# jabhinav/RetinaNet-for-Table-Detection

Hardware: AMD Instinct MI355X
Metric: images/sec RetinaNet R50-FPN 800x1333 inference (higher is better)
Workload: dtype bf16; 1 GPU; ResNet50-FPN RetinaNet inference 800x1333 bf16 batch 8/GPU incl. decode+NMS (BASELINE.json configs[1]); batch_per_gpu=8, anchors_per_image=200700, parallelism=dp1 (images sharded, no collective), batches_in_flight=2

## Files before the change

retinanet-for-table-detection_amd/csrc/rtn_conv_halon.hip:

```cpp
#include "rtn_internal.h"
#include "rtn_device.h"

namespace {

typedef __attribute__((ext_vector_type(8))) __bf16 bf16x8;
typedef __attribute__((ext_vector_type(4))) float f32x4;
typedef __attribute__((ext_vector_type(4))) unsigned u32x4;

constexpr unsigned HN_OOB = 0xFFFFFF00u;
constexpr int HN_THREADS = 512;
constexpr int HN_R = 256, HN_TM = HN_R - 3;
constexpr unsigned HN_HALO = 32768, HN_ZERO_ROW = (HN_R - 1) * 128u;

template <int NF>
struct HNCfg {
    static constexpr int BR = 48 * NF;
    static constexpr int BP = BR / 8;
    static constexpr int BPW = (BP + 7) / 8;
    static constexpr unsigned STAGE = HN_HALO + BR * 128u;
    static constexpr unsigned DUMP = 3 * STAGE;
    static constexpr int LDS = 3 * (int)STAGE + 1024;
    static constexpr int PP = 4 + BPW;
};

struct HNGroup {
    const char* in;
    char* out;
    unsigned in_bytes, out_bytes;
    int Hin, Win, M, tile_begin;
    int in_row_stride_b;
    int cells;
    unsigned out_img_stride, out_off;
    float inv_cells, inv_w;
};

struct HNParams {
    HNGroup g[RTN_MAX_GROUPS];
    const char* w;
    const float* bias;
    unsigned w_bytes;
    int ngroups, ntiles;
    int N, Kbytes, nchunk, pad_t, pad_l, relu, sigmoid, out_ld, pix_b, vec, xcd, kh_fast;
};

__device__ __forceinline__ void dma16(const i32x4& srd, unsigned voff, unsigned soff, unsigned lds_addr) {
    unsigned keep;
    const unsigned la = (unsigned)__builtin_amdgcn_readfirstlane((int)lds_addr), so = (unsigned)__builtin_amdgcn_readfirstlane((int)soff);
    asm volatile("s_mov_b32 %0, m0\n\ts_mov_b32 m0, %2\n\ts_nop 0\n\tbuffer_load_dwordx4 %1, %3, %4 offen lds\n\ts_mov_b32 m0, %0"
                 : "=&s"(keep)
                 : "v"(voff), "s"(la), "s"(srd), "s"(so)
                 : "memory");
}

#define RTN_STORE_GUARD(V) asm volatile("s_nop 3" :: "v"(V.x), "v"(V.y), "v"(V.z), "v"(V.w));
#define RTN_STORE_GUARD1(V) asm volatile("s_nop 1" :: "v"(V));

template <int NF>
__global__ __launch_bounds__(HN_THREADS, 2) void conv_halon_kernel(const HNParams p) {
    typedef HNCfg<NF> Cfg;
    extern __shared__ __attribute__((aligned(16))) char lds[];

    const int t = threadIdx.x, lane = t & 63;
    const int wave = __builtin_amdgcn_readfirstlane(t >> 6);
    const int lr = lane >> 3, sc = (lane & 7) ^ lr;
    const int lrow = lane & 15, kq = lane >> 4;
    const unsigned lds_base = (unsigned)(size_t)(__attribute__((address_space(3))) char*)lds;
    const int nchunk = p.nchunk;
    const int G = 3 * nchunk;
    const i32x4 w_srd = make_srd(p.w, p.w_bytes);

    unsigned wvoff[Cfg::BPW];
#pragma unroll
    for (int d = 0; d < Cfg::BPW; ++d) {
        const int row = (d * 8 + wave) * 8 + lr;
        const int kw = row / (16 * NF), n = row - kw * (16 * NF);
        wvoff[d] = row < Cfg::BR ? (unsigned)n * (unsigned)p.Kbytes + (unsigned)(kw * nchunk * 128) + (unsigned)sc * 16u : HN_OOB;
    }

    unsigned hbase[4];
    int hiy[4];
    i32x4 in_srd = w_srd;
    int st_Hin = 1, st_row_b = 0;
    auto stage_tile = [&](int T) {
        if (T >= p.ntiles) {
#pragma unroll
            for (int i = 0; i < 4; ++i) { hiy[i] = -(1 << 28); hbase[i] = 0; }
            return;
        }
        int gi = 0;
#pragma unroll
        for (int i = 1; i < RTN_MAX_GROUPS; ++i)
            if (i < p.ngroups && T >= p.g[i].tile_begin) gi = i;
        const HNGroup& Gs = p.g[gi];
        const int m0 = (T - Gs.tile_begin) * HN_TM;
        in_srd = make_srd(Gs.in, Gs.in_bytes);
        st_Hin = Gs.Hin;
        st_row_b = Gs.in_row_stride_b;
#pragma unroll
        for (int i = 0; i < 4; ++i) {
            const int h = (i * 8 + wave) * 8 + lr;
            const int f = m0 + h - p.pad_l;
            if (h < HN_R - 1 && f >= 0 && f < Gs.M) {
                int b, rem, y, x;
                divmod24(f, Gs.cells, Gs.inv_cells, b, rem);
                divmod24(rem, Gs.Win, Gs.inv_w, y, x);
                hiy[i] = y;
                hbase[i] = (unsigned)f * (unsigned)p.pix_b + (unsigned)sc * 16u;
            } else {
                hiy[i] = -(1 << 28);
                hbase[i] = 0;
            }
        }
    };
    auto tile_of = [&](int v) {
        if (v >= p.ntiles || !p.xcd) return v;
        const int x = v & 7, j = v >> 3, base = p.ntiles >> 3, rem = p.ntiles & 7;
        return x * base + (x < rem ? x : rem) + j;
    };
    int st_v = blockIdx.x, st_kh = 0, st_cc = 0;
    unsigned st_ring = 0;
#define HN_ISSUE(I)                                                                                            \
    if ((I) < 4) {                                                                                             \
        const int dy_ = st_kh - p.pad_t;                                                                       \
        const unsigned delta_ = (unsigned)(dy_ * st_row_b + st_cc * 128);                                      \
        const bool ok_ = (unsigned)(hiy[(I) & 3] + dy_) < (unsigned)st_Hin;                                    \
        dma16(in_srd, ok_ ? hbase[(I) & 3] + delta_ : HN_OOB, 0u, lds_base + st_ring + (unsigned)(wave * 1024 + ((I) & 3) * 8192)); \
    } else if ((I) < Cfg::PP) {                                                                                \
        constexpr int d_ = (I) >= 4 && (I) - 4 < Cfg::BPW ? (I) - 4 : 0;                                       \
        const unsigned kcol_ = (unsigned)((st_kh * 3 * nchunk + st_cc) * 128);                                 \
        const int P_ = d_ * 8 + wave;                                                                          \
        dma16(w_srd, wvoff[d_], kcol_, lds_base + (P_ < Cfg::BP ? st_ring + HN_HALO + (unsigned)P_ * 1024u : Cfg::DUMP)); \
    }
    auto advance_stage = [&]() {
        st_ring = st_ring == 2 * Cfg::STAGE ? 0u : st_ring + Cfg::STAGE;
        if (p.kh_fast) {
            if (++st_kh == 3) {
                st_kh = 0;
                if (++st_cc == nchunk) { st_cc = 0; st_v += (int)gridDim.x; stage_tile(tile_of(st_v)); }
            }
        } else if (++st_cc == nchunk) {
            st_cc = 0;
            if (++st_kh == 3) {
                st_kh = 0;
                st_v += (int)gridDim.x;
                stage_tile(tile_of(st_v));
            }
        }
    };
    auto issue_stage = [&]() {
        HN_ISSUE(0) HN_ISSUE(1) HN_ISSUE(2) HN_ISSUE(3) HN_ISSUE(4) HN_ISSUE(5) HN_ISSUE(6)
        advance_stage();
    };

    f32x4 bias4[NF];
#pragma unroll
    for (int f = 0; f < NF; ++f) {
        bias4[f] = (f32x4){0.f, 0.f, 0.f, 0.f};
        if (p.bias) bias4[f] = *reinterpret_cast<const f32x4*>(p.bias + 16 * f + 4 * kq);
    }
    const unsigned w_lane = HN_HALO + (unsigned)(lrow * 128 + ((kq ^ (lrow & 7)) << 4));

    stage_tile(tile_of(st_v));
    issue_stage();
    issue_stage();

    unsigned c_ring = 0;
    int cv = blockIdx.x;
    bool first = true;
    while (cv < p.ntiles) {
        const int tile = tile_of(cv);
        int gi = 0;
#pragma unroll
        for (int i = 1; i < RTN_MAX_GROUPS; ++i)
            if (i < p.ngroups && tile >= p.g[i].tile_begin) gi = i;
        const HNGroup& Gc = p.g[gi];
        const int m0 = (tile - Gc.tile_begin) * HN_TM;
        unsigned arow[3][2];
        unsigned obase[2];
#pragma unroll
        for (int i = 0; i < 2; ++i) {
            const int rloc = wave * 32 + i * 16 + lrow;
            const int m = m0 + rloc;
            const int mc = m < Gc.M ? m : Gc.M - 1;
            int b, rem, y, x;
            divmod24(mc, Gc.cells, Gc.inv_cells, b, rem);
            divmod24(rem, Gc.Win, Gc.inv_w, y, x);
#pragma unroll
            for (int kw = 0; kw < 3; ++kw) {
                const int rr = rloc + kw;
                const bool off = rloc >= HN_TM || (unsigned)(x + kw - p.pad_l) >= (unsigned)Gc.Win;
                arow[kw][i] = off ? HN_ZERO_ROW : (unsigned)(rr * 128 + ((kq ^ (rr & 7)) << 4));
            }
            obase[i] = (rloc < HN_TM && m < Gc.M) ? (unsigned)b * Gc.out_img_stride + Gc.out_off + (unsigned)rem * (unsigned)p.out_ld : HN_OOB;
        }
        f32x4 acc[2][NF];
#pragma unroll
        for (int i = 0; i < 2; ++i)
#pragma unroll
            for (int f = 0; f < NF; ++f) acc[i][f] = bias4[f];

#pragma unroll 1
        for (int g = 0; g < G; ++g) {
            if (g == 0 && !first) {
                if (p.vec) asm volatile("s_waitcnt vmcnt(%0)" :: "n"(Cfg::PP + 2 * NF) : "memory");
                else       asm volatile("s_waitcnt vmcnt(%0)" :: "n"(Cfg::PP + 8 * NF) : "memory");
            } else {
                asm volatile("s_waitcnt vmcnt(%0)" :: "n"(Cfg::PP) : "memory");
            }
            __builtin_amdgcn_s_barrier();
            const char* sb = lds + c_ring;
            uint4 fx[2][2], fw[2][NF];
#define HN_READ(STEP, SET)                                                                                     \
            {                                                                                                  \
                const int kw_ = ((STEP) >> 1) % 3;                                                             \
                const unsigned ks_ = ((STEP) & 1) * 64u;                                                       \
                _Pragma("unroll") for (int i = 0; i < 2; ++i) fx[SET][i] = *reinterpret_cast<const uint4*>(sb + (arow[kw_][i] ^ ks_)); \
                _Pragma("unroll") for (int f = 0; f < NF; ++f)                                                 \
                    fw[SET][f] = *reinterpret_cast<const uint4*>(sb + ((w_lane ^ ks_) + (unsigned)((kw_ * NF + f) * 2048))); \
            }
#define HN_STEP(STEP)                                                                                          \
            {                                                                                                  \
                if ((STEP) + 1 < 6) HN_READ((STEP) + 1, ((STEP) + 1) & 1)                                      \
                if (0 * 6 / Cfg::PP == (STEP)) { HN_ISSUE(0) }                                                 \
                if (1 * 6 / Cfg::PP == (STEP)) { HN_ISSUE(1) }                                                 \
                if (2 * 6 / Cfg::PP == (STEP)) { HN_ISSUE(2) }                                                 \
                if (3 * 6 / Cfg::PP == (STEP)) { HN_ISSUE(3) }                                                 \
                if (4 * 6 / Cfg::PP == (STEP)) { HN_ISSUE(4) }                                                 \
                if (5 < Cfg::PP && 5 * 6 / Cfg::PP == (STEP)) { HN_ISSUE(5) }                                  \
                if (6 < Cfg::PP && 6 * 6 / Cfg::PP == (STEP)) { HN_ISSUE(6) }                                  \
                _Pragma("unroll") for (int f = 0; f < NF; ++f)                                                 \
                    _Pragma("unroll") for (int i = 0; i < 2; ++i)                                              \
                        acc[i][f] = __builtin_amdgcn_mfma_f32_16x16x32_bf16(__builtin_bit_cast(bf16x8, fw[(STEP) & 1][f]),      \
                                                                           __builtin_bit_cast(bf16x8, fx[(STEP) & 1][i]), acc[i][f], 0, 0, 0); \
            }
            HN_READ(0, 0)
            HN_STEP(0) HN_STEP(1) HN_STEP(2) HN_STEP(3) HN_STEP(4) HN_STEP(5)
#undef HN_STEP
#undef HN_READ
            advance_stage();
            c_ring = c_ring == 2 * Cfg::STAGE ? 0u : c_ring + Cfg::STAGE;
        }
        {
            const __amdgpu_buffer_rsrc_t out_rsrc = __builtin_amdgcn_make_buffer_rsrc(
                (void*)Gc.out, 0, (int)__builtin_amdgcn_readfirstlane((int)Gc.out_bytes), 0x00020000);
#pragma unroll
            for (int i = 0; i < 2; ++i)
#pragma unroll
                for (int f = 0; f < NF; ++f) {
                    f32x4 v = acc[i][f];
                    if (p.relu) {
#pragma unroll
                        for (int r = 0; r < 4; ++r) v[r] = v[r] > 0.f ? v[r] : 0.f;
                    }
                    if (p.sigmoid) {
#pragma unroll
                        for (int r = 0; r < 4; ++r) v[r] = 1.0f / (1.0f + expf(-v[r]));
                    }
                    const int ch0 = 16 * f + 4 * kq;
                    const int cnt = p.N - ch0;
                    if (p.vec) {
                        const unsigned off = (obase[i] != HN_OOB && cnt >= 4) ? (obase[i] + (unsigned)ch0) * 4u : HN_OOB;
                        u32x4 o = __builtin_bit_cast(u32x4, v);
                        __builtin_amdgcn_raw_buffer_store_b128(o, out_rsrc, (int)off, 0, 0);
                        RTN_STORE_GUARD(o)
                    } else {
#pragma unroll
                        for (int r = 0; r < 4; ++r) {
                            const unsigned off = (obase[i] != HN_OOB && r < cnt) ? (obase[i] + (unsigned)(ch0 + r)) * 4u : HN_OOB;
                            const unsigned o = __float_as_uint(v[r]);
                            __builtin_amdgcn_raw_buffer_store_b32(o, out_rsrc, (int)off, 0, 0);
                            RTN_STORE_GUARD1(o)
                        }
                    }
                }
        }
        cv += (int)gridDim.x;
        first = false;
    }
    asm volatile("s_waitcnt vmcnt(0)" ::: "memory");
#undef HN_ISSUE
}

}

int rtn_conv_halon_try(rtn_handle_t h, const rtn_conv_desc_t* d, int grid_limit, bool forced) {
    if (d->dtype != RTN_BF16) return 1;
    if (d->KW != 3 || d->KH != 3 || d->sy != 1 || d->sx != 1) return 1;
    if (!(d->flags & RTN_CONV_OUT_F32) || (d->flags & ~(RTN_CONV_OUT_F32 | RTN_CONV_RELU | RTN_CONV_SIGMOID))) return 1;
    if (d->N < 1 || d->N > 48 || d->out_ld < d->N) return 1;
    const int nf = (d->N + 15) / 16;
    if (d->w_rows < 16 * nf) return 1;
    if (d->Crun != d->pix_stride || (d->Crun * 2) % 128 || d->Crun <= 0) return 1;
    if (d->pad_l < 0 || d->pad_l >= 3 || d->pad_t < 0 || d->pad_t >= 3) return 1;
    if (((uintptr_t)d->w & 15) || ((uintptr_t)d->bias & 15)) return 1;
    const int nchunk = d->Crun * 2 / 128;
    const long long Kbytes = 9ll * d->Crun * 2;
    if (Kbytes * d->w_rows >= 0xFFFFFF00ll) return 1;
    HNParams p;
    memset(&p, 0, sizeof(p));
    const int cus = h->num_cus > 0 ? h->num_cus : 256;
    long long tiles = 0;
    bool vec = d->N % 4 == 0 && d->out_ld % 4 == 0;
    for (int i = 0; i < d->ngroups; ++i) {
        const rtn_conv_group_t& s = d->g[i];
        if (s.Hin != s.Hout || s.Win != s.Wout || s.in_row_stride != (long long)s.Win * d->pix_stride ||
            s.in_img_stride != (long long)s.Hin * s.in_row_stride) return 1;
        const long long cells = (long long)s.Hout * s.Wout, M = cells * d->batch;
        if (s.out_step > 1 || s.out_off < 0 || M >= (1ll << 24) || M < 1) return 1;
        if (!s.in || !s.out || ((uintptr_t)s.in & 15) || ((uintptr_t)s.out & 3)) return 1;
        if (s.in_elems < M * d->Crun || s.in_elems * 2 >= 0xFFFFFF00ll || s.out_elems * 4 >= 0xFFFFFF00ll) return 1;
        if (s.out_img_stride < 0 || (d->batch - 1) * s.out_img_stride + s.out_off + (cells - 1) * d->out_ld + d->N > s.out_elems) return 1;
        if (((uintptr_t)s.out & 15) || s.out_img_stride % 4 || s.out_off % 4) vec = false;
        HNGroup& g = p.g[i];
        g.in = (const char*)s.in;
        g.out = (char*)s.out;
        g.in_bytes = (unsigned)(s.in_elems * 2);
        g.out_bytes = (unsigned)(s.out_elems * 4);
        g.Hin = s.Hin; g.Win = s.Win; g.M = (int)M;
        g.cells = (int)cells;
        g.tile_begin = (int)tiles;
        g.in_row_stride_b = (int)(s.in_row_stride * 2);
        g.out_img_stride = (unsigned)s.out_img_stride;
        g.out_off = (unsigned)s.out_off;
        g.inv_cells = 1.0f / (float)cells;
        g.inv_w = 1.0f / (float)s.Win;
        tiles += (M + HN_TM - 1) / HN_TM;
    }
    if (tiles < 1 || tiles > 0x3fffffff) return 1;
    if (!forced && tiles * 4 < cus) return 1;
    p.w = (const char*)d->w;
    p.bias = d->bias;
    p.w_bytes = (unsigned)(Kbytes * d->w_rows);
    p.ngroups = d->ngroups;
    p.ntiles = (int)tiles;
    p.N = d->N;
    p.Kbytes = (int)Kbytes;
    p.nchunk = nchunk;
    p.pad_t = d->pad_t; p.pad_l = d->pad_l;
    p.relu = (d->flags & RTN_CONV_RELU) ? 1 : 0;
    p.sigmoid = (d->flags & RTN_CONV_SIGMOID) ? 1 : 0;
    p.out_ld = d->out_ld;
    p.pix_b = d->pix_stride * 2;
    p.vec = vec ? 1 : 0;
    p.xcd = 1;
    p.kh_fast = 1;
    int grid = cus;
    if (grid_limit > 0 && grid_limit < grid) grid = grid_limit;
    if (grid > p.ntiles) grid = p.ntiles;
    const dim3 gdim((unsigned)grid), bdim(HN_THREADS);
    const int lrc = nf == 1 ? rtn_launch_lds<conv_halon_kernel<1>>(h, gdim, bdim, HNCfg<1>::LDS, HNCfg<1>::LDS, p)
                  : nf == 2 ? rtn_launch_lds<conv_halon_kernel<2>>(h, gdim, bdim, HNCfg<2>::LDS, HNCfg<2>::LDS, p)
                            : rtn_launch_lds<conv_halon_kernel<3>>(h, gdim, bdim, HNCfg<3>::LDS, HNCfg<3>::LDS, p);
    if (lrc != RTN_OK) return lrc;
    RTN_CHECK_LAUNCH(h, "conv_halon_kernel");
    return RTN_OK;
}
```

Measured before the change: 2441 images/sec.

## Add 2D-tiled halo conv kernel for 3x3 head convolutions

Adds a new 3x3 convolution kernel that tiles the output as 2D blocks (8x32 or 6x42 pixels) with a small halo, in place of 1D row strips that stage a large halo. Per output tile the kernel double-buffers the halo input across channel chunks and streams the weights per kh-row into LDS, overlapping DMA with the MFMA work. The aim is to cut redundant halo loads and LDS footprint, which could allow two blocks per CU. It is enabled by default through an env flag, and it adds complex index math plus the risk of partially filled tiles at the image edges.

Result: no change. 2440 images/sec (-0.0%).

```diff
diff --git a/retinanet-for-table-detection_amd/csrc/rtn_conv_halon.hip b/retinanet-for-table-detection_amd/csrc/rtn_conv_halon.hip
--- a/retinanet-for-table-detection_amd/csrc/rtn_conv_halon.hip
+++ b/retinanet-for-table-detection_amd/csrc/rtn_conv_halon.hip
@@ -32,6 +32,8 @@
     int cells;
     unsigned out_img_stride, out_off;
     float inv_cells, inv_w;
+    int th, tw, txn, tpi;
+    float inv_tw, inv_hw, inv_txn, inv_tpi;
 };
 
 struct HNParams {
@@ -281,6 +283,255 @@
 #undef HN_ISSUE
 }
 
+constexpr int H2_HJ = 6;
+constexpr int H2_PIECES = 44;
+constexpr unsigned H2_HALO = H2_PIECES * 1024u;
+struct H2Shape { int th, tw; };
+constexpr H2Shape H2_SHAPES[] = {{8, 32}, {6, 42}};
+constexpr bool h2_shapes_fit() {
+    for (const H2Shape& s : H2_SHAPES)
+        if (s.th * s.tw > 256 || (s.th + 2) * (s.tw + 2) > H2_PIECES * 8) return false;
+    return true;
+}
+static_assert(h2_shapes_fit(), "a tile is at most 256 pixels and its halo at most one halo slot");
+
+template <int NF>
+struct H2Cfg {
+    static constexpr int BR = 48 * NF, BP = BR / 8, BPW = (BP + 7) / 8;
+    static constexpr unsigned WST = BR * 128u;
+    static constexpr unsigned WBASE = 2 * H2_HALO;
+    static constexpr unsigned DUMP = WBASE + 3 * WST;
+    static constexpr int LDS = (int)DUMP + 1024;
+};
+
+template <int NF>
+__global__ __launch_bounds__(HN_THREADS, 2) void conv_halon2d_kernel(const HNParams p) {
+    typedef H2Cfg<NF> Cfg;
+    extern __shared__ __attribute__((aligned(16))) char lds[];
+
+    const int t = threadIdx.x, lane = t & 63;
+    const int wave = __builtin_amdgcn_readfirstlane(t >> 6);
+    const int lr = lane >> 3, sc = (lane & 7) ^ lr;
+    const int lrow = lane & 15, kq = lane >> 4;
+    const unsigned lds_base = (unsigned)(size_t)(__attribute__((address_space(3))) char*)lds;
+    const int nchunk = p.nchunk;
+    const i32x4 w_srd = make_srd(p.w, p.w_bytes);
+
+    unsigned wvoff[Cfg::BPW];
+#pragma unroll
+    for (int d = 0; d < Cfg::BPW; ++d) {
+        const int row = (d * 8 + wave) * 8 + lr;
+        const int kw = row / (16 * NF), n = row - kw * (16 * NF);
+        wvoff[d] = row < Cfg::BR ? (unsigned)n * (unsigned)p.Kbytes + (unsigned)(kw * nchunk * 128) + (unsigned)sc * 16u : HN_OOB;
+    }
+
+    unsigned hbase[H2_HJ];
+    i32x4 in_srd = w_srd;
+    auto stage_tile = [&](int T) {
+        if (T >= p.ntiles) {
+#pragma unroll
+            for (int j = 0; j < H2_HJ; ++j) hbase[j] = HN_OOB;
+            return;
+        }
+        int gi = 0;
+#pragma unroll
+        for (int i = 1; i < RTN_MAX_GROUPS; ++i)
+            if (i < p.ngroups && T >= p.g[i].tile_begin) gi = i;
+        const HNGroup& Gs = p.g[gi];
+        int b, r, ty, tx;
+        divmod24(T - Gs.tile_begin, Gs.tpi, Gs.inv_tpi, b, r);
+        divmod24(r, Gs.txn, Gs.inv_txn, ty, tx);
+        const int y0 = ty * Gs.th - p.pad_t, x0 = tx * Gs.tw - p.pad_l, hw = Gs.tw + 2, hrows = (Gs.th + 2) * hw;
+        in_srd = make_srd(Gs.in, Gs.in_bytes);
+#pragma unroll
+        for (int j = 0; j < H2_HJ; ++j) {
+            const int h = (j * 8 + wave) * 8 + lr;
+            int hy, hx;
+            divmod24(h, hw, Gs.inv_hw, hy, hx);
+            const int iy = y0 + hy, ix = x0 + hx;
+            const bool ok = h < hrows && (unsigned)iy < (unsigned)Gs.Hin && (unsigned)ix < (unsigned)Gs.Win;
+            hbase[j] = ok ? (unsigned)((b * Gs.Hin + iy) * Gs.Win + ix) * (unsigned)p.pix_b + (unsigned)sc * 16u : HN_OOB;
+        }
+    };
+    auto tile_of = [&](int v) {
+        if (v >= p.ntiles || !p.xcd) return v;
+        const int x = v & 7, j = v >> 3, base = p.ntiles >> 3, rem = p.ntiles & 7;
+        return x * base + (x < rem ? x : rem) + j;
+    };
+#define H2_HALO_PIECE(J, CC, HB)                                                                               \
+    {                                                                                                          \
+        const int P_ = (J) * 8 + wave;                                                                         \
+        dma16(in_srd, hbase[J] != HN_OOB ? hbase[J] + (unsigned)((CC) * 128) : HN_OOB, 0u,                     \
+              lds_base + (P_ < H2_PIECES ? (HB) + (unsigned)P_ * 1024u : Cfg::DUMP));                          \
+    }
+#define H2_W_PIECE(D, FKH, FCC)                                                                                \
+    {                                                                                                          \
+        const unsigned kcol_ = (unsigned)(((FKH) * 3 * nchunk + (FCC)) * 128);                                 \
+        const int P_ = (D) * 8 + wave;                                                                         \
+        dma16(w_srd, wvoff[D], kcol_, lds_base + (P_ < Cfg::BP ? Cfg::WBASE + (FKH) * Cfg::WST + (unsigned)P_ * 1024u : Cfg::DUMP)); \
+    }
+#define H2_ISSUE(KH, I)                                                                                        \
+    if ((KH) < 2 && (I) < 3) {                                                                                 \
+        constexpr int j_ = ((KH) < 2 && (I) < 3) ? (KH) * 3 + (I) : 0;                                         \
+        H2_HALO_PIECE(j_, ncc, hb ^ H2_HALO)                                                                   \
+    } else if ((I) - ((KH) < 2 ? 3 : 0) < Cfg::BPW) {                                                          \
+        constexpr int d0_ = (I) - ((KH) < 2 ? 3 : 0);                                                          \
+        constexpr int d_ = d0_ >= 0 && d0_ < Cfg::BPW ? d0_ : 0;                                               \
+        constexpr int fkh_ = ((KH) + 2) % 3;                                                                   \
+        const int fcc_ = (KH) == 0 ? c : ncc;                                                                  \
+        H2_W_PIECE(d_, fkh_, fcc_)                                                                             \
+    }
+
+    f32x4 bias4[NF];
+#pragma unroll
+    for (int f = 0; f < NF; ++f) {
+        bias4[f] = (f32x4){0.f, 0.f, 0.f, 0.f};
+        if (p.bias) bias4[f] = *reinterpret_cast<const f32x4*>(p.bias + 16 * f + 4 * kq);
+    }
+    const unsigned w_lane = Cfg::WBASE + (unsigned)(lrow * 128 + ((kq ^ (lrow & 7)) << 4));
+
+    int st_v = blockIdx.x;
+    unsigned hb = 0;
+    stage_tile(tile_of(st_v));
+    H2_HALO_PIECE(0, 0, 0u) H2_HALO_PIECE(1, 0, 0u) H2_HALO_PIECE(2, 0, 0u)
+    H2_HALO_PIECE(3, 0, 0u) H2_HALO_PIECE(4, 0, 0u) H2_HALO_PIECE(5, 0, 0u)
+#pragma unroll
+    for (int d = 0; d < Cfg::BPW; ++d) H2_W_PIECE(d, 0, 0)
+#pragma unroll
+    for (int d = 0; d < Cfg::BPW; ++d) H2_W_PIECE(d, 1, 0)
+
+    int cv = blockIdx.x;
+    bool first = true;
+    while (cv < p.ntiles) {
+        const int tile = tile_of(cv);
+        int gi = 0;
+#pragma unroll
+        for (int i = 1; i < RTN_MAX_GROUPS; ++i)
+            if (i < p.ngroups && tile >= p.g[i].tile_begin) gi = i;
+        const HNGroup& Gc = p.g[gi];
+        int tb, trem, ty, tx;
+        divmod24(tile - Gc.tile_begin, Gc.tpi, Gc.inv_tpi, tb, trem);
+        divmod24(trem, Gc.txn, Gc.inv_txn, ty, tx);
+        const int hw = Gc.tw + 2, tpix = Gc.th * Gc.tw;
+        unsigned arow[3][3][2];
+        unsigned obase[2];
+#pragma unroll
+        for (int i = 0; i < 2; ++i) {
+            const int rloc = wave * 32 + i * 16 + lrow;
+            const int rc = rloc < tpix ? rloc : tpix - 1;
+            int y, x;
+            divmod24(rc, Gc.tw, Gc.inv_tw, y, x);
+            const int oy = ty * Gc.th + y, ox = tx * Gc.tw + x;
+#pragma unroll
+            for (int kh = 0; kh < 3; ++kh)
+#pragma unroll
+                for (int kw = 0; kw < 3; ++kw) {
+                    const int hp = (y + kh) * hw + x + kw;
+                    arow[kh][kw][i] = (unsigned)(hp * 128 + ((kq ^ (hp & 7)) << 4));
+                }
+            obase[i] = (rloc < tpix && oy < Gc.Hin && ox < Gc.Win)
+                           ? (unsigned)tb * Gc.out_img_stride + Gc.out_off + (unsigned)(oy * Gc.Win + ox) * (unsigned)p.out_ld : HN_OOB;
+        }
+        f32x4 acc[2][NF];
+#pragma unroll
+        for (int i = 0; i < 2; ++i)
+#pragma unroll
+            for (int f = 0; f < NF; ++f) acc[i][f] = bias4[f];
+
+#pragma unroll 1
+        for (int c = 0; c < nchunk; ++c) {
+            int ncc = c + 1;
+            if (ncc == nchunk) { ncc = 0; st_v += (int)gridDim.x; stage_tile(tile_of(st_v)); }
+            const char* hbuf = lds + hb;
+#define H2_READ(KH, STEP, SET)                                                                                 \
+            {                                                                                                  \
+                constexpr int kw_ = (STEP) >> 1;                                                               \
+                constexpr unsigned ks_ = ((STEP) & 1) * 64u;                                                   \
+                _Pragma("unroll") for (int i = 0; i < 2; ++i) fx[SET][i] = *reinterpret_cast<const uint4*>(hbuf + (arow[KH][kw_][i] ^ ks_)); \
+                _Pragma("unroll") for (int f = 0; f < NF; ++f)                                                 \
+                    fw[SET][f] = *reinterpret_cast<const uint4*>(lds + ((w_lane ^ ks_) + (unsigned)((KH) * Cfg::WST + (kw_ * NF + f) * 2048))); \
+            }
+#define H2_STEP(KH, STEP)                                                                                      \
+            {                                                                                                  \
+                constexpr int pp_ = ((KH) < 2 ? 3 : 0) + Cfg::BPW;                                             \
+                if ((STEP) + 1 < 6) H2_READ(KH, ((STEP) + 1) % 6, ((STEP) + 1) & 1)                            \
+                if (0 * 6 / pp_ == (STEP)) { H2_ISSUE(KH, 0) }                                                 \
+                if (1 < pp_ && 1 * 6 / pp_ == (STEP)) { H2_ISSUE(KH, 1) }                                      \
+                if (2 < pp_ && 2 * 6 / pp_ == (STEP)) { H2_ISSUE(KH, 2) }                                      \
+                if (3 < pp_ && 3 * 6 / pp_ == (STEP)) { H2_ISSUE(KH, 3) }                                      \
+                if (4 < pp_ && 4 * 6 / pp_ == (STEP)) { H2_ISSUE(KH, 4) }                                      \
+                if (5 < pp_ && 5 * 6 / pp_ == (STEP)) { H2_ISSUE(KH, 5) }                                      \
+                _Pragma("unroll") for (int f = 0; f < NF; ++f)                                                 \
+                    _Pragma("unroll") for (int i = 0; i < 2; ++i)                                              \
+                        acc[i][f] = __builtin_amdgcn_mfma_f32_16x16x32_bf16(__builtin_bit_cast(bf16x8, fw[(STEP) & 1][f]),      \
+                                                                           __builtin_bit_cast(bf16x8, fx[(STEP) & 1][i]), acc[i][f], 0, 0, 0); \
+            }
+#define H2_GROUP(KH)                                                                                           \
+            {                                                                                                  \
+                if ((KH) == 0) {                                                                               \
+                    if (c == 0 && !first) {                                                                    \
+                        if (p.vec) asm volatile("s_waitcnt vmcnt(%0)" :: "n"(Cfg::BPW + 2 * NF) : "memory");   \
+                        else       asm volatile("s_waitcnt vmcnt(%0)" :: "n"(Cfg::BPW + 8 * NF) : "memory");   \
+                    } else {                                                                                   \
+                        asm volatile("s_waitcnt vmcnt(%0)" :: "n"(Cfg::BPW) : "memory");                       \
+                    }                                                                                          \
+                } else {                                                                                       \
+                    asm volatile("s_waitcnt vmcnt(%0)" :: "n"(3 + Cfg::BPW) : "memory");                       \
+                }                                                                                              \
+                __builtin_amdgcn_s_barrier();                                                                  \
+                uint4 fx[2][2], fw[2][NF];                                                                     \
+                H2_READ(KH, 0, 0)                                                                              \
+                H2_STEP(KH, 0) H2_STEP(KH, 1) H2_STEP(KH, 2) H2_STEP(KH, 3) H2_STEP(KH, 4) H2_STEP(KH, 5)      \
+            }
+            H2_GROUP(0) H2_GROUP(1) H2_GROUP(2)
+#undef H2_GROUP
+#undef H2_STEP
+#undef H2_READ
+            hb ^= H2_HALO;
+        }
+        {
+            const __amdgpu_buffer_rsrc_t out_rsrc = __builtin_amdgcn_make_buffer_rsrc(
+                (void*)Gc.out, 0, (int)__builtin_amdgcn_readfirstlane((int)Gc.out_bytes), 0x00020000);
+#pragma unroll
+            for (int i = 0; i < 2; ++i)
+#pragma unroll
+                for (int f = 0; f < NF; ++f) {
+                    f32x4 v = acc[i][f];
+                    if (p.relu) {
+#pragma unroll
+                        for (int r = 0; r < 4; ++r) v[r] = v[r] > 0.f ? v[r] : 0.f;
+                    }
+                    if (p.sigmoid) {
+#pragma unroll
+                        for (int r = 0; r < 4; ++r) v[r] = 1.0f / (1.0f + expf(-v[r]));
+                    }
+                    const int ch0 = 16 * f + 4 * kq;
+                    const int cnt = p.N - ch0;
+                    if (p.vec) {
+                        const unsigned off = (obase[i] != HN_OOB && cnt >= 4) ? (obase[i] + (unsigned)ch0) * 4u : HN_OOB;
+                        u32x4 o = __builtin_bit_cast(u32x4, v);
+                        __builtin_amdgcn_raw_buffer_store_b128(o, out_rsrc, (int)off, 0, 0);
+                        RTN_STORE_GUARD(o)
+                    } else {
+#pragma unroll
+                        for (int r = 0; r < 4; ++r) {
+                            const unsigned off = (obase[i] != HN_OOB && r < cnt) ? (obase[i] + (unsigned)(ch0 + r)) * 4u : HN_OOB;
+                            const unsigned o = __float_as_uint(v[r]);
+                            __builtin_amdgcn_raw_buffer_store_b32(o, out_rsrc, (int)off, 0, 0);
+                            RTN_STORE_GUARD1(o)
+                        }
+                    }
+                }
+        }
+        cv += (int)gridDim.x;
+        first = false;
+    }
+    asm volatile("s_waitcnt vmcnt(0)" ::: "memory");
+#undef H2_ISSUE
+#undef H2_W_PIECE
+#undef H2_HALO_PIECE
+}
+
 }
 
 int rtn_conv_halon_try(rtn_handle_t h, const rtn_conv_desc_t* d, int grid_limit, bool forced) {
@@ -299,7 +550,8 @@
     HNParams p;
     memset(&p, 0, sizeof(p));
     const int cus = h->num_cus > 0 ? h->num_cus : 256;
-    long long tiles = 0;
+    const bool two_d = rtn_env_int("RTN_HALON_2D", 1) != 0;
+    long long tiles = 0, tiles2 = 0;
     bool vec = d->N % 4 == 0 && d->out_ld % 4 == 0;
     for (int i = 0; i < d->ngroups; ++i) {
         const rtn_conv_group_t& s = d->g[i];
@@ -318,16 +570,32 @@
         g.out_bytes = (unsigned)(s.out_elems * 4);
         g.Hin = s.Hin; g.Win = s.Win; g.M = (int)M;
         g.cells = (int)cells;
-        g.tile_begin = (int)tiles;
+        g.tile_begin = (int)(two_d ? tiles2 : tiles);
         g.in_row_stride_b = (int)(s.in_row_stride * 2);
         g.out_img_stride = (unsigned)s.out_img_stride;
         g.out_off = (unsigned)s.out_off;
         g.inv_cells = 1.0f / (float)cells;
         g.inv_w = 1.0f / (float)s.Win;
         tiles += (M + HN_TM - 1) / HN_TM;
+        long long best = 0;
+        for (const H2Shape& sh : H2_SHAPES) {
+            const long long tyn = (s.Hout + sh.th - 1) / sh.th, txn = (s.Wout + sh.tw - 1) / sh.tw;
+            if (best && tyn * txn >= best) continue;
+            best = tyn * txn;
+            g.th = sh.th; g.tw = sh.tw; g.txn = (int)txn; g.tpi = (int)best;
+        }
+        g.inv_tw = 1.0f / (float)g.tw;
+        g.inv_hw = 1.0f / (float)(g.tw + 2);
+        g.inv_txn = 1.0f / (float)g.txn;
+        g.inv_tpi = 1.0f / (float)g.tpi;
+        tiles2 += best * d->batch;
     }
     if (tiles < 1 || tiles > 0x3fffffff) return 1;
     if (!forced && tiles * 4 < cus) return 1;
+    if (two_d) {
+        if (tiles2 >= (1ll << 24)) return 1;
+        tiles = tiles2;
+    }
     p.w = (const char*)d->w;
     p.bias = d->bias;
     p.w_bytes = (unsigned)(Kbytes * d->w_rows);
@@ -348,10 +616,13 @@
     if (grid_limit > 0 && grid_limit < grid) grid = grid_limit;
     if (grid > p.ntiles) grid = p.ntiles;
     const dim3 gdim((unsigned)grid), bdim(HN_THREADS);
-    const int lrc = nf == 1 ? rtn_launch_lds<conv_halon_kernel<1>>(h, gdim, bdim, HNCfg<1>::LDS, HNCfg<1>::LDS, p)
+    const int lrc = two_d ? (nf == 1 ? rtn_launch_lds<conv_halon2d_kernel<1>>(h, gdim, bdim, H2Cfg<1>::LDS, H2Cfg<1>::LDS, p)
+                           : nf == 2 ? rtn_launch_lds<conv_halon2d_kernel<2>>(h, gdim, bdim, H2Cfg<2>::LDS, H2Cfg<2>::LDS, p)
+                                     : rtn_launch_lds<conv_halon2d_kernel<3>>(h, gdim, bdim, H2Cfg<3>::LDS, H2Cfg<3>::LDS, p))
+                  : nf == 1 ? rtn_launch_lds<conv_halon_kernel<1>>(h, gdim, bdim, HNCfg<1>::LDS, HNCfg<1>::LDS, p)
                   : nf == 2 ? rtn_launch_lds<conv_halon_kernel<2>>(h, gdim, bdim, HNCfg<2>::LDS, HNCfg<2>::LDS, p)
                             : rtn_launch_lds<conv_halon_kernel<3>>(h, gdim, bdim, HNCfg<3>::LDS, HNCfg<3>::LDS, p);
     if (lrc != RTN_OK) return lrc;
-    RTN_CHECK_LAUNCH(h, "conv_halon_kernel");
+    RTN_CHECK_LAUNCH(h, two_d ? "conv_halon2d_kernel" : "conv_halon_kernel");
     return RTN_OK;
 }
```
